# aschneuw/road-segmentation-unet

Measured on AMD Instinct MI355X. Metric: 388x388 patches/sec fwd+bwd (1/2/4/8 GPU) + conv MFMA % of peak, higher is better.
Workload: dtype bf16; 1 GPU; U-Net fwd+bwd+momentum step, num_layers=5 root_size=64 patch_size=388 input=572; batch_per_gpu=4, global_batch=4, parallelism=dp1

## Files before the change

road_segmentation_unet_amd/_lib.py:

```python
import ctypes
import os

_HERE = os.path.dirname(os.path.abspath(__file__))
LIB_PATH = os.environ.get("RSU_LIB_PATH") or os.path.join(_HERE, "librsu_hip.so")

_vp, _i, _l, _f, _sz, _u = ctypes.c_void_p, ctypes.c_int, ctypes.c_long, ctypes.c_float, ctypes.c_size_t, ctypes.c_uint


class RsuSrc(ctypes.Structure):
    _fields_ = [("ptr", _vp), ("H", _i), ("W", _i), ("C", _i), ("oy", _i), ("ox", _i)]


class RsuWgradJob(ctypes.Structure):
    _fields_ = [("kind", _i), ("src", RsuSrc), ("dz", _vp), ("dw", _vp), ("db", _vp), ("Ho", _i), ("Wo", _i),
                ("Cin_total", _i), ("ci_off", _i), ("Cout", _i), ("dil", _i)]


WGRAD_CONV3X3, WGRAD_CONVT2X2, WGRAD_GROUP_MAX = 0, 1, 16


class RsuPlanRow(ctypes.Structure):
    _fields_ = [(n, _i) for n in ("kind", "level", "Hin", "Win", "Cin", "Hout", "Wout", "Cout", "dilation", "nsrc")]


# ... 135 lines not shown
    "rsu_lovasz_ws_bytes": (_sz, [_i, _i, _i]),
    "rsu_lovasz_fwd": (_i, [_vp, _vp, _vp, _vp, _i, _i, _i, _vp]),
    "rsu_lovasz_fwd_bwd": (_i, [_vp, _vp, _f, _i, _vp, _vp, _vp, _i, _i, _i, _vp]),
}

SIGNATURES_COMPONENTS = {
    "rsu_components_ws_bytes": (_sz, [_i, _i, _i]),
    "rsu_components_label": (_i, [_vp, _f, _i, _i, _vp, _vp, _vp, _vp, _i, _i, _i, _vp]),
    "rsu_components_filter": (_i, [_vp, _f, _i, _i, _i, _vp, _vp, _vp, _i, _i, _i, _vp]),
    "rsu_components_pair_count": (_i, [_vp, _f, _vp, _i, _vp, _vp, _i, _i, _i, _vp]),
}

SIGNATURES_DISTANCE = {
    "rsu_distance_ws_bytes": (_sz, [_i, _i, _i]),
    "rsu_mask_distance": (_i, [_vp, _f, _vp, _vp, _vp, _vp, _i, _i, _i, _vp]),
    "rsu_distance_hist": (_i, [_vp, _f, _vp, _vp, _vp, _i, _i, _i, _vp]),
}

SIGNATURES_THIN = {
    "rsu_thin_ws_bytes": (_sz, [_i, _i, _i, _i]),
    "rsu_mask_thin": (_i, [_vp, _f, _vp, _i, _vp, _vp, _vp, _vp, _vp, _i, _i, _i, _vp]),
}

_lib = None


class RsuError(RuntimeError):
    pass


def lib():
    global _lib
    if _lib is None:
        if not os.path.exists(LIB_PATH):
            raise RsuError("HIP extension missing: %s (build it with `python -c 'import __graft_entry__ as g; g.build()'` "
                           "or `make -C road_segmentation_unet_amd/csrc`); there is no fallback path" % LIB_PATH)
        L = ctypes.CDLL(LIB_PATH)
        for name, (res, args) in list(SIGNATURES.items()) + list(SIGNATURES_OPTIM.items()) + list(SIGNATURES_LOSS.items()) \
                + list(SIGNATURES_CLDICE.items()) + list(SIGNATURES_LOVASZ.items()) + list(SIGNATURES_COMPONENTS.items()) \
                + list(SIGNATURES_DISTANCE.items()) + list(SIGNATURES_THIN.items()):
            fn = getattr(L, name)
            fn.restype = res
            fn.argtypes = args
        _lib = L
    return _lib


TUNE_OFF, TUNE_LOOKUP, TUNE_MEASURE = 0, 1, 2
EVAL_BINS = 256
BORDER_D2_INF, BORDER_MAX_SIDE = 0x7fffffff, 1024
CLIP_STATE_BYTES, CLIP_CLIPPED, CLIP_NONFINITE, GRAD_NORM_BLOCK_FLOATS = 32, 1, 2, 16384
GRAD_ACCUMULATE_BLOCK_FLOATS = 8192
DECAY_L2, DECAY_DECOUPLED = 0, 1
AFFINE_MAX_LAUNCH = 32
ELASTIC_MAX_LAUNCH, ELASTIC_MAX_GRID = 32, 16
JITTER_MAX_LAUNCH = 32
CLDICE_MAX_ITERS = 16
DIST_BINS, DIST_NONE, DIST_MAX_SIDE = 64, 0x7fffffff, 1024
THIN_MAX_SIDE, THIN_MAX_ITERS = 1024, 512
E2BIG = -7


def check(rc, what):
# ... 73 lines not shown
```

road_segmentation_unet_amd/csrc/igemm.h:

```cpp
#pragma once
#include "rsu_common.h"

struct IgSrc {
    const bf16_t* ptr;
    int H, W, C;
    int oy, ox;
};

struct IgFwdParams {
    IgSrc src[3];
    int nsrc;
    int nchunk[3];
    const bf16_t* wp;
    long wp_y_stride;
    int ntiles_w;
    int tile_off;
    const float* bias;
    bf16_t* out;
    const bf16_t* mask_src;
    bf16_t* pool_out;
    unsigned char* pool_code;
    const void* zero_page;
    int N, Hin, Win;
    int Ho, Wo;
// ... 30 lines not shown
hipError_t igemm_pp_finish_launch(int cfg, const IgFwdParams& p, hipStream_t st);

struct IgCtParams {
    const bf16_t* a;
    int Ca;
    int nchunk;
    int N, H, W;
    unsigned magic_hw, magic_w;
    const bf16_t* wp;
    long wp_phase_stride;
    int ntiles_w;
    const float* bias;
    bf16_t* out;
    int outC;
    int Cn;
    const bf16_t* mask_src;
    int ncob, nnb;
};
bool igemm_ct_supports(int mode, int N, int H, int W, int Ca, int Cn);
hipError_t igemm_ct_launch(int mode, const IgCtParams& p, int grid_x, hipStream_t st);
hipError_t conv_first_fwd_launch(const void* in16, const void* wp, int ntiles_w, const float* bias, void* y, int N, int H, int W, int Cout, int dil,
                                 int relu, int ncu, hipStream_t st, const float* x = nullptr, const float* cw = nullptr, const float* cb = nullptr);

struct IgWgradParams {
    const bf16_t* F;
    int Hf, Wf, Cf;
    IgSrc S;
    float* slab;
    float* bslab;
    float* sbslab;
    long slab_stride;
    int CsOut, CfOut, cs_off;
    const void* zero_page;
    int N, dil, stride;
    int nsplit, ntiles_total;
    int lsw;
    int nbuf, nsw;
    int dbg;
    TileGeo g;
};
enum { IGW_CFG_64x64 = 0, IGW_CFG_64x16 = 1, IGW_CFG_128x64 = 2, IGW_NCFG = 3 };
size_t igemm_wgrad_lds_bytes(int cfg, int npix_max, int nbuf);
int igemm_wgrad_nsw(int cfg, int npix_max);
int igemm_wgrad_tmk(int cfg);
int igemm_wgrad_cfb(int cfg);
int igemm_wgrad_csb(int cfg);
int igemm_wgrad_kgroups(int cfg);
hipError_t igemm_wgrad_launch(int cfg, int ntap, const IgWgradParams& p, int grid_x, int grid_y, int grid_z,
                              hipStream_t st);
bool igemm_wgt_supports(int N, int H, int W, int Cin, int Cout);
int igemm_wgt_blocks(int Cin, int Cout);
int igemm_wgt_tiles(int N, int H, int W);
hipError_t igemm_wgt_launch(const void* x, const void* dy, float* slab, float* sbslab, long slab_stride, int N, int H, int W, int Cin, int Cout,
                            int nsplit, hipStream_t st);
bool igemm_wg1_supports(int N, int H, int W, int Cout, int dil);
int igemm_wg1_blocks(int Cout);
int igemm_wg1_tiles(int N, int Ho, int Wo);
hipError_t igemm_wg1_launch(const void* in16, const void* dz, float* slab, float* bslab, long slab_stride, int N, int H, int W, int Cout, int dil,
                            int nsplit, hipStream_t st);
enum { IGW_FAM_WGPP3 = 0, IGW_FAM_WGPP4 = 1, IGW_FAM_WGPP5 = 2, IGW_FAM_WGPP6 = 3, IGW_FAM_WGP64_4 = 4, IGW_FAM_WGP64_5 = 5,
       IGW_FAM_GENERIC = 8  };
#define IGW_GROUP_MAX 16
// ... 22 lines not shown
```

road_segmentation_unet_amd/csrc/igemm_wgpp.hip:

```cpp
#include <type_traits>

#include "igemm_wgrad_body.h"

#define RSU_SENT 0x80000000u

namespace {
constexpr int sched_nph(int sch) { return sch >= 4 ? 1 : 2; }
constexpr int sched_count(int sch, int ph) {
    constexpr int T2[8] = {0, 3, 0, 3, 0, 3, 0, 0}, T1[4] = {3, 3, 3, 0};
    return sch >= 4 ? T1[ph] : T2[ph];
}
constexpr int sched_first(int sch, int ph) {
    int n = 0;
    for (int i = 0; i < ph; ++i) n += sched_count(sch, i);
    return n;
}
#ifndef WGPP_NT
#define WGPP_NT 0
#endif
#ifndef WG64_NT
#define WG64_NT 0
#endif
template <int NT = 0>
__device__ __forceinline__ void bdma16w(__amdgpu_buffer_rsrc_t rsrc, unsigned voff, unsigned soff, void* lds_wave_base) {
// ... 539 lines not shown
#pragma unroll
                for (int ct = 0; ct < CFT; ++ct) {
                    const int cf = cfb * 64 + ((ct + wcs) & 3) * 16 + 4 * g4;
                    if (cf >= p.Cf) continue;
                    float* dst = p.slab + (long)z * p.slab_stride + (((long)(T0 + t) * p.CsOut + p.cs_off + cs) * p.CfOut + cf);
                    *(f32x4*)dst = acc[t][ct];
                }
            }
        }
    };
    if (grp) {
        run(I1{});
    } else {
        run(I0{});
        bar();
    }
    asm volatile("s_waitcnt vmcnt(0)" ::: "memory");
}

#define WG_UNIT_FROM_GRID()                                                                                                                   \
    extern __shared__ __attribute__((aligned(16))) char smem[];                                                                              \
    __attribute__((address_space(3))) char* lds = (__attribute__((address_space(3))) char*)smem;                                             \
    const int lid = xcd_contiguous_id(blockIdx.x + gridDim.x * (blockIdx.y + gridDim.y * blockIdx.z), gridDim.x * gridDim.y * gridDim.z);  \
    const int cfb = lid % gridDim.x, csb = (lid / gridDim.x) % gridDim.y, z = lid / (gridDim.x * gridDim.y)
template <int LSW, int DBG, int SCH>
__global__ void __launch_bounds__(512) __attribute__((amdgpu_waves_per_eu(2, 2))) igemm_wgpp_kernel(const IgWgradParams p) {
    WG_UNIT_FROM_GRID();
    igemm_wgpp_body<LSW, DBG, SCH>(p, lds, cfb, csb, z, threadIdx.x);
}
template <int LSW>
__global__ void __launch_bounds__(512) __attribute__((amdgpu_waves_per_eu(2, 2))) igemm_wgp64_kernel(const IgWgradParams p) {
    WG_UNIT_FROM_GRID();
    igemm_wgp64_body<LSW>(p, lds, cfb, csb, z, threadIdx.x);
}

template <int FAM, class P>
__device__ __forceinline__ void wg_group_unit(const P& p, __attribute__((address_space(3))) char* lds, int cfb, int csb, int z, unsigned tid) {
    if constexpr (FAM == IGW_FAM_WGPP3) igemm_wgpp_body<3, 0, 4>(p, lds, cfb, csb, z, tid);
    else if constexpr (FAM == IGW_FAM_WGPP4) igemm_wgpp_body<4, 0, 4>(p, lds, cfb, csb, z, tid);
    else if constexpr (FAM == IGW_FAM_WGPP5) igemm_wgpp_body<5, 0, 4>(p, lds, cfb, csb, z, tid);
    else if constexpr (FAM == IGW_FAM_WGPP6) igemm_wgpp_body<6, 0, 4>(p, lds, cfb, csb, z, tid);
    else if constexpr (FAM == IGW_FAM_WGP64_4) igemm_wgp64_body<4>(p, lds, cfb, csb, z, tid);
    else if constexpr (FAM == IGW_FAM_WGP64_5) igemm_wgp64_body<5>(p, lds, cfb, csb, z, tid);
    else {
        constexpr int CFG = (FAM - IGW_FAM_GENERIC) >> 1, NTAP = ((FAM - IGW_FAM_GENERIC) & 1) ? 4 : 9, KW = NTAP == 4 ? 2 : 3;
        using C = WgCfg<CFG>;
        igemm_wgrad_body<C::WCF, C::WCS, C::CFT, C::CST, NTAP, KW, C::TMK, C::KG>(p, lds, cfb, csb, z, tid);
    }
}
__global__ void __launch_bounds__(512) __attribute__((amdgpu_waves_per_eu(2, 2))) igemm_wg_group_kernel(const IgWgGroupParams* table) {
    extern __shared__ __attribute__((aligned(16))) char smem[];
    __attribute__((address_space(3))) char* lds = (__attribute__((address_space(3))) char*)smem;
    {
        const unsigned state = IGW_GROUP_LDS_BYTES - 256 + (threadIdx.x >> 6) * 16;
        const u32x4 st0 = {(unsigned)__ldg(&table->wg_first[blockIdx.x]), (unsigned)__ldg(&table->wg_first[blockIdx.x + 1]),
                           (unsigned)(uintptr_t)table, (unsigned)((uintptr_t)table >> 32)};
// ... 125 lines not shown
```

road_segmentation_unet_amd/csrc/igemm_wgrad.hip:

```cpp
#include "igemm_wgrad_body.h"

template <int WCF, int WCS, int CFT, int CST, int NTAP, int KW, int TMK, int KG>
__global__ void __launch_bounds__(WCF* WCS * KG * 64) __attribute__((amdgpu_waves_per_eu(WCF* WCS* KG / 4, WCF* WCS* KG / 4)))
igemm_wgrad_kernel(const IgWgradParams p) {
    extern __shared__ __attribute__((aligned(16))) char smem[];
    __attribute__((address_space(3))) char* lds = (__attribute__((address_space(3))) char*)smem;
    const int lid = xcd_contiguous_id(blockIdx.x + gridDim.x * (blockIdx.y + gridDim.y * blockIdx.z), gridDim.x * gridDim.y * gridDim.z);
    const int cfb = lid % gridDim.x, csb = (lid / gridDim.x) % gridDim.y, z = lid / (gridDim.x * gridDim.y);
    igemm_wgrad_body<WCF, WCS, CFT, CST, NTAP, KW, TMK, KG>(p, lds, cfb, csb, z, threadIdx.x);
}

int igemm_wgrad_kgroups(int) { return 1; }
int igemm_wgrad_tmk(int) { return 128; }
int igemm_wgrad_cfb(int cfg) { return cfg == IGW_CFG_128x64 ? 128 : 64; }
int igemm_wgrad_csb(int cfg) { return cfg == IGW_CFG_64x16 ? 16 : 64; }

int igemm_wgrad_nsw(int cfg, int npix_max) {
    const int csb = igemm_wgrad_csb(cfg);
    const int ppp = 64 / (csb / 8);
    return ((npix_max + ppp - 1) / ppp + 7) / 8;
}
size_t igemm_wgrad_lds_bytes(int cfg, int npix_max, int nbuf) {
    const int csb = igemm_wgrad_csb(cfg);
    const size_t staging = (size_t)nbuf * igemm_wgrad_tmk(cfg) * 2 * igemm_wgrad_cfb(cfg) +
                           (size_t)nbuf * igemm_wgrad_nsw(cfg, npix_max) * 8 * 1024;
    const size_t reduce = cfg == IGW_CFG_128x64 ? 0 : (size_t)(9 * 64 * csb + 64 * csb) * 4;
    return staging > reduce ? staging : reduce;
}

template <int CFG, int NTAP, int KW>
static hipError_t wlaunch_one(const IgWgradParams& p, int gx, int gy, int gz, hipStream_t st) {
    using C = WgCfg<CFG>;
// ... 25 lines not shown
```

road_segmentation_unet_amd/csrc/igemm_wgrad_body.h:

```cpp
#pragma once
#include "igemm.h"


static __device__ __forceinline__ void bdma16(__amdgpu_buffer_rsrc_t rsrc, unsigned voff, unsigned soff, void* lds_wave_base) {
    __builtin_amdgcn_raw_ptr_buffer_load_lds(rsrc, (__attribute__((address_space(3))) void*)lds_wave_base, 16, voff, soff, 0, 0);
}
#define RSU_WG_WAIT(N) asm volatile("s_waitcnt vmcnt(%0)" ::"n"(N) : "memory")
#define RSU_SENT 0x80000000u

template <int WCF, int WCS, int CFT, int CST, int NTAP, int KW, int TMK, int KG, class P>
__device__ __forceinline__ void igemm_wgrad_body(const P& p, __attribute__((address_space(3))) char* lds, const int cfb, const int csb,
                                                 const int z, const unsigned tid) {
    constexpr int NW = WCF * WCS * KG;
    constexpr int KS = TMK / 32;
    constexpr int KSG = KS / KG;
    static_assert(KS % KG == 0, "k-steps must split evenly over the wave groups");
    constexpr int CFB = WCF * CFT * 16;
    constexpr int NPL = CFB / 64;
    constexpr int CSB = WCS * CST * 16;
    constexpr int KH = NTAP / KW;
    constexpr int SPITCH = CSB * 2;
    constexpr int LPP = CSB / 8;
    constexpr int PPP = 64 / LPP;
    constexpr int FPL = TMK * 128;
    constexpr int FBUF = NPL * FPL;
    static_assert(CFB % 64 == 0, "F block is a multiple of 64 channels");
    const int nbuf = p.nbuf, nsw = p.nsw;
    const int SBUF = nsw * NW * 1024;
    const int s_base = nbuf * FBUF;

    const int lane = tid & 63;
// ... 374 lines not shown
```

road_segmentation_unet_amd/csrc/rsu_api.hip:

```cpp
#include <array>
#include <atomic>
#include <cmath>
#include <cstdlib>
#include <cstring>
#include <algorithm>
#include <cstddef>
#include <map>
#include <mutex>
#include <vector>

#include "../../include/rsu.h"
#include "../../include/rsu_optim.h"
#include "../../include/rsu_loss.h"
#include "../../include/rsu_cldice.h"
#include "../../include/rsu_lovasz.h"
#include "../../include/rsu_components.h"
#include "../../include/rsu_distance.h"
#include "../../include/rsu_thin.h"
#include "affine_patches.h"
#include "color_jitter.h"
#include "border_map.h"
#include "elementwise.h"
#include "head.h"
#include "cldice.h"
#include "lovasz.h"
#include "components.h"
#include "distance.h"
#include "thin.h"
#include "optim.h"
#include "igemm.h"

static std::atomic<int> g_last_hip_error{0};
static void rsu_set_hip_error(int e) { g_last_hip_error.store(e); }

__device__ uint4 g_zero_page_dev[256];

static const void* zero_page() {
    static void* ptr[64] = {nullptr};
    int dev = 0;
    if (hipGetDevice(&dev) != hipSuccess || dev < 0 || dev >= 64) return nullptr;
    if (!ptr[dev]) {
// ... 949 lines not shown
    p.nsplit = pl.nsplit;
    p.ntiles_total = pl.ntiles;
    p.lsw = pl.lsw;
    p.nbuf = pl.nbuf;
    p.nsw = igemm_wgrad_nsw(cfg, pl.g.npix_max);
#ifdef RSU_DEV_KERNELS
    p.dbg = env_int("RSU_WG_DBG", 0);
#endif
    p.g = pl.g;
    w.cfg = cfg; w.ntap = ntap; w.gx = pl.gx; w.gy = pl.gy; w.ntiles = pl.ntiles;
    w.main_elems = (long)ntap * CsOut * CfOut;
    w.extra = db ? CfOut : (dbs ? rup(CsOut, 4) : 0);
    w.out = out; w.db = db; w.dbs = dbs; w.cs_cnt = S->C;
    return RSU_OK;
}
static void finish_wgrad(WgPrep& w, int nsplit, float* ws) {
    IgWgradParams& p = w.p;
    p.nsplit = nsplit;
    p.slab = nsplit == 1 ? w.out : ws;
    p.slab_stride = w.main_elems + w.extra;
    p.bslab = w.db ? (nsplit == 1 ? w.db : ws + w.main_elems) : nullptr;
    p.sbslab = w.dbs ? (nsplit == 1 ? w.dbs : ws + w.main_elems) : nullptr;
}
static int run_wgrad(int cfg, const void* F, int Hf, int Wf, int Cf, const rsu_src_t* S, float* out, float* ws, int CsOut, int CfOut,
                     int cs_off, int N, int ntap, int kw, int dil, int stride, int ncu_arg, hipStream_t st, float* db = nullptr, float* dbs = nullptr) {
    const int ncu = launch_ncu(ncu_arg);
    if (ncu < 0) return RSU_EINVAL;
    WgPrep w;
    const int rc = prep_wgrad(w, cfg, F, Hf, Wf, Cf, S, out, CsOut, CfOut, cs_off, N, ntap, kw, dil, stride, ncu, db, dbs);
    if (rc != RSU_OK) return rc;
    const int nslab = w.p.nsplit;
    finish_wgrad(w, nslab, ws);
    const IgWgradParams& p = w.p;
    if (env_int("RSU_WG_GEN", 2) >= 2 && igemm_wgpp_supports(w.cfg, ntap, p))
        HIP_CHECK_RET(igemm_wgpp_launch(p, w.gx, w.gy, nslab, st));
    else if (env_int("RSU_WG_GEN", 2) >= 2 && env_int("RSU_WG64", 1) && igemm_wgp64_supports(w.cfg, ntap, p))
        HIP_CHECK_RET(igemm_wgp64_launch(p, w.gx, w.gy, nslab, st));
    else
        HIP_CHECK_RET(igemm_wgrad_launch(w.cfg, ntap, p, w.gx, w.gy, nslab, st));
    if (nslab > 1) {
        HIP_CHECK_RET(ew_reduce_slabs(ws, out, db ? db : dbs, w.extra / 4, nslab, p.slab_stride, ntap, CsOut, cs_off, S->C, CfOut, st));
    }
    return RSU_OK;
}

extern "C" size_t rsu_conv2d_bwd_weight_ws_floats(int Cin_total, int src_C, int Cout) {
    return wgrad_max_slabs(IGW_CFG_64x64, Cout, src_C) * (9 * (size_t)Cin_total * Cout + Cout);
}
extern "C" int rsu_conv2d_bwd_weight(const rsu_src_t* src, const void* dz, float* dw, float* db, float* ws, int N, int Ho, int Wo,
                                     int Cin_total, int ci_off, int Cout, int dil, int ncu, rsu_stream_t stream) {
    if (!src || !src->ptr || !dz || !dw || !ws || src->C % 8 || Cout % 8 || ci_off + src->C > Cin_total || (dil != 1 && dil != 2))
        return RSU_EINVAL;
    if (src->oy < 0 || src->ox < 0 || src->oy + Ho + 2 * dil > src->H || src->ox + Wo + 2 * dil > src->W || Wo < 2) return RSU_EINVAL;
    return run_wgrad(IGW_CFG_64x64, dz, Ho, Wo, Cout, src, dw, ws, Cin_total, Cout, ci_off, N, 9, 3, dil, 1, ncu, (hipStream_t)stream, db);
}

extern "C" size_t rsu_convT2x2_bwd_weight_ws_floats(int Cin, int Cout) {
    size_t slabs = wgrad_max_slabs(IGW_CFG_64x64, Cin, Cout);
    const size_t wgt = (size_t)(256 / igemm_wgt_blocks(Cin, Cout));
    if (wgt > slabs) slabs = wgt;
    return slabs * (4 * (size_t)Cout * Cin + Cout);
}
extern "C" int rsu_convT2x2_bwd_weight(const void* x, const void* dy, float* dK, float* db, float* ws, int N, int H, int W, int Cin,
                                       int Cout, int ncu, rsu_stream_t stream) {
    if (!x || !dy || !dK || !ws || Cin % 8 || Cout % 8 || W < 2) return RSU_EINVAL;
    const int wgt_gen = env_int("RSU_WGT_GEN", 3);
    if (wgt_gen >= 2 && igemm_wgt_supports(N, H, W, Cin, Cout) && (wgt_gen >= 3 || launch_ncu(ncu) >= 192)) {
        const int n = launch_ncu(ncu);
        if (n < 0) return RSU_EINVAL;
        const int ntiles = igemm_wgt_tiles(N, H, W);
        int nsplit = n / igemm_wgt_blocks(Cin, Cout);
        nsplit = nsplit < 1 ? 1 : (nsplit > ntiles ? ntiles : nsplit);
        const long main_elems = 4l * Cout * Cin, extra = db ? rup(Cout, 4) : 0, stride = main_elems + extra;
        HIP_CHECK_RET(igemm_wgt_launch(x, dy, nsplit == 1 ? dK : ws, db ? (nsplit == 1 ? db : ws + main_elems) : nullptr, stride, N, H, W, Cin, Cout,
                                       nsplit, (hipStream_t)stream));
        if (nsplit > 1) HIP_CHECK_RET(ew_reduce_slabs(ws, dK, db, (int)(extra / 4), nsplit, stride, 4, Cout, 0, Cout, Cin, (hipStream_t)stream));
        return RSU_OK;
// ... 706 lines not shown
```

road_segmentation_unet_amd/unet.py:

```python
import ctypes
import math
import os

import numpy as np
import torch

from . import _lib
from ._lib import RsuSrc, RsuWgradJob, call
from .optim import (DECAY_MODES, DEFAULT_LR_SCHEDULE, EMA_SUFFIX, LR_SCHEDULES, OPTIMIZERS, OptimizerStep,
                    _PACK_CONV_BWD, _PACK_CONV_FIRST, _PACK_CONV_FWD, _PACK_CONVT_BWD, _PACK_CONVT_FWD, _accumulate_arg, _clip_arg,
                    _decay_args, _ema_arg, _int_arg, _ptr, adam_scalars, clip_scale, ema_decay_at, lr_at)
from .schedule import BackwardSchedule, cu_shares

NUM_CHANNELS = 3
NUM_LABELS = 2


def input_size_needed(output_size, num_layers):
    for i in range(num_layers - 1):
        assert output_size % 2 == 0, 'expand layer {} has size {} not divisible by 2' \
            .format(num_layers - i, output_size)
        output_size = (output_size + 4) / 2
    for i in range(num_layers - 1):
        output_size = (output_size + 4) * 2
# ... 22 lines not shown
    shapes += [("weight_output/kernel", (1, 1, nf, NUM_LABELS)), ("weight_output/bias", (NUM_LABELS,))]
    return shapes


def _is_dead(name, num_layers):
    return name.startswith("conv_dilut_%d/" % (num_layers - 1))


def glorot_uniform_params(num_layers, root_size, dilated_layers, seed):
    rng = np.random.RandomState(seed)
    out = {}
    for name, shp in param_shapes(num_layers, root_size, dilated_layers):
        if name.endswith("kernel"):
            recept = shp[0] * shp[1]
            limit = math.sqrt(6.0 / (recept * shp[2] + recept * shp[3]))
            out[name] = rng.uniform(-limit, limit, size=shp).astype(np.float32)
        else:
            out[name] = np.zeros(shp, np.float32)
    return out


def dropout_key_value(seed, site, global_step, micro_step=0):
    return (seed * 0x9E3779B9 + site * 0x85EBCA6B + global_step * 0xC2B2AE35 + micro_step * 0x27D4EB2F) & 0xFFFFFFFF


def _src(t, h, w):
    H, W, C = t.shape[1], t.shape[2], t.shape[3]
    return RsuSrc(t.data_ptr(), H, W, C, (H - h) // 2, (W - w) // 2)


class UNet(OptimizerStep):

    def __init__(self, num_layers, root_size, dilated_layers, batch_size, patch_size, device="cuda:0", params=None, seed=2017,
                 training=True, optimizer="momentum", class_weights=None, dice_weight=0.0, dice_smooth=1.0, border_weight=0.0, border_sigma=5.0,
                 clip_grad_norm=None, ema_decay=None, ema_warmup=True, accumulate_steps=None, weight_decay=None, weight_decay_mode="decoupled",
                 focal_gamma=0.0, cldice_weight=0.0, cldice_iters=10, cldice_smooth=1.0, lovasz_weight=0.0):
        self._init_optimizer(training, optimizer, clip_grad_norm, ema_decay, ema_warmup, accumulate_steps, weight_decay, weight_decay_mode)
        assert root_size % 8 == 0 and (root_size // 8) & (root_size // 8 - 1) == 0, "root_size must be 8 * 2^k for the HIP path"
        self.L, self.root, self.dilated = num_layers, root_size, bool(dilated_layers)
        self.B, self.P = batch_size, patch_size
        self.S = input_size_needed(patch_size, num_layers)
        self.device = torch.device(device)
        if self.device.type == "cuda":
            torch.cuda.set_device(self.device)
        self.training = training
        self.class_weights = class_weights
# ... 278 lines not shown
                h = (h - 4) // 2
                nf *= 2
        h = h - 4
        for i in range(L - 1):
            nf //= 2
            j = L + i
            self.act["up_%d" % i] = self._bf(B, 2 * h, 2 * h, nf)
            h = 2 * h
            self.act["c1_%d" % j] = self._bf(B, h - 2, h - 2, nf)
            self.act["c2_%d" % j] = self._bf(B, h - 4, h - 4, nf)
            h -= 4
        assert h == self.P, (h, self.P)
        self.last_name = "c2_%d" % (2 * L - 2) if L > 1 else "c2_0"
        self.prob = torch.zeros((B, self.P, self.P), dtype=torch.float32, device=dev)
        self.logits = torch.zeros((B, self.P, self.P, 2), dtype=torch.float32, device=dev)
        self.labels = torch.zeros((B, self.P, self.P), dtype=torch.int64, device=dev)
        self._loss_acc = torch.zeros(2, dtype=torch.float32, device=dev)
        self.loss_sum, self.weight_sum = self._loss_acc[0:1], self._loss_acc[1:2]
        self.dice_sums = torch.zeros(3, dtype=torch.float32, device=dev)
        self.eval_sums = torch.zeros(5, dtype=torch.float32, device=dev)
        self.eval_hist = torch.zeros((2, _lib.EVAL_BINS), dtype=torch.int64, device=dev)
        nk = int(_lib.lib().rsu_conv_splitk_ws_floats()) if os.environ.get("RSU_KSPLIT", "1") != "0" else 0
        self.sched.kws = torch.zeros(nk, dtype=torch.float32, device=dev) if nk else None
        self.sched.kws_side = [torch.zeros(nk, dtype=torch.float32, device=dev) for _ in self.wstreams] if (nk and self.dilated) else []
        if self.training:
            for k, t in self.act.items():
                if k.startswith("up_") or k.startswith("c") or k.startswith("d") or k.startswith("pool_"):
                    self.grad[k] = torch.zeros_like(t)
            for i in range(L - 1):
                up = self.act["up_%d" % i]
                self.grad["skip_%d" % i] = torch.zeros_like(up)
                if self.dilated:
                    self.grad["skipd_%d" % i] = torch.zeros_like(up)
            lib = _lib.lib()
            ws = [lib.rsu_head_ws_floats(B * self.P * self.P, self.root), lib.rsu_head_w_ws_floats(B * self.P * self.P, self.root),
                  lib.rsu_head_dice_ws_floats(B * self.P * self.P, self.root), lib.rsu_head_eval_ws_floats(B * self.P * self.P, self.root),
                  lib.rsu_conv_first_bwd_ws_floats(self.root)]
            for kind, n, s, segs in self._packed_kernels():
                if kind == _PACK_CONV_FWD:
                    for c in segs:
                        ws.append(lib.rsu_conv2d_bwd_weight_ws_floats(s[2], c, s[3]))
                    ws.append(lib.rsu_bias_grad_ws_floats(B * S * S, s[3]))
                elif kind == _PACK_CONVT_FWD:
                    ws.append(lib.rsu_convT2x2_bwd_weight_ws_floats(s[3], s[2]))
            ws.append(lib.rsu_wgrad_group_ws_floats())
            self.ws = torch.zeros(int(max(ws)) + 64, dtype=torch.float32, device=dev)
            self.sched.ws_side = [self.ws] + [torch.zeros_like(self.ws) for _ in self.wstreams[1:]]
            self.gfirst = torch.zeros((2, 9, 12, self.root), dtype=torch.float32, device=dev)
            if self._cldice_weight > 0.0:
                self._cldice_buffers()
            if self._lovasz_weight > 0.0:
                self._lovasz_buffers()
            if self.border_weight > 0.0:
                self.border_map = torch.zeros((B, self.P, self.P), dtype=torch.float32, device=dev)
                self._border_ws = torch.zeros(int(lib.rsu_border_map_ws_bytes(B, self.P, self.P)) // 4, dtype=torch.int32, device=dev)
            if os.environ.get("RSU_POOL_CODE", "1") == "1":
                for i in range(L - 1):
                    self.pool_code[i] = torch.zeros(self.act["pool_%d" % i].shape, dtype=torch.uint8, device=dev)

    def _conv_sources_c(self, name, shape):
        cin, cout = shape[2], shape[3]
        blk = int(name.split("/")[0].split("_")[-1]) if name.startswith("conv_") and not name.startswith("conv_dilut") else -1
        if name.endswith("conv1/kernel") and blk >= self.L:
            return [cout] * (3 if self.dilated else 2)
# ... 191 lines not shown
            self.eval_lovasz_sum.zero_()

    def evaluate_device(self):
        if not self.training:
            raise _lib.RsuError("evaluate_device needs a training net (labels and the head's workspace); a forward-only net has no loss")
        if self.keep != 1.0:
            raise _lib.RsuError("evaluate_device follows forward_device(keep=1.0): the activations in flight were made with dropout")
        if self._focal_gamma > 0.0:
            call("rsu_head_eval_focal", _ptr(self.act[self.last_name]), _ptr(self.w["weight_output/kernel"]), _ptr(self.w["weight_output/bias"]),
                 _ptr(self.labels), _ptr(self._class_w_dev), _ptr(self._head_pixel_weights()), self._focal_gamma, _ptr(self.prob),
                 _ptr(self.eval_sums), _ptr(self.eval_hist), _ptr(self.ws), self.B * self.P * self.P, self.root, self._stream())
        else:
            call("rsu_head_eval", _ptr(self.act[self.last_name]), _ptr(self.w["weight_output/kernel"]), _ptr(self.w["weight_output/bias"]),
                 _ptr(self.labels), _ptr(self._class_w_dev), _ptr(self._head_pixel_weights()), _ptr(self.prob), _ptr(self.eval_sums),
                 _ptr(self.eval_hist), _ptr(self.ws), self.B * self.P * self.P, self.root, self._stream())
        if self._cldice_weight > 0.0:
            self._cldice_buffers()
            self._cldice_fwd(self.eval_cldice_sums)
        if self._lovasz_weight > 0.0:
            self._lovasz_buffers()
            call("rsu_lovasz_fwd", _ptr(self.prob), _ptr(self.labels), _ptr(self.eval_lovasz_sum), _ptr(self._lovasz_ws), self.B, self.P,
                 self.P, self._stream())

    def _wgrad(self, name, srcs_t, dz, hout, dil=1, block_done=False):
        cout = dz.shape[3]
        cin_total = self.w[name + "/kernel"].shape[2]
        off = 0
        if self.sched.grouped:
            for t, win in srcs_t:
                db = self.g[name + "/bias"] if off == 0 else None
                job = RsuWgradJob(_lib.WGRAD_CONV3X3, _src(t, win, win), dz.data_ptr(), self.g[name + "/kernel"].data_ptr(),
                                  db.data_ptr() if db is not None else None, hout, hout, cin_total, off, cout, dil)
                self.sched.queue(job, 2.0 * self.B * hout * hout * cout * t.shape[3] * 9, (name, off))
                off += t.shape[3]
            if block_done:
                self.sched.block_done()
            return
        with self.sched.side() as ws:
            st = self._stream()
            for t, win in srcs_t:
                s = _src(t, win, win)
                db = _ptr(self.g[name + "/bias"]) if off == 0 else None
                fl = 2.0 * self.B * hout * hout * cout * t.shape[3] * 9
                self._timed("conv3x3_bwd_weight", fl, "rsu_conv2d_bwd_weight", ctypes.byref(s), _ptr(dz), _ptr(self.g[name + "/kernel"]), db,
                            _ptr(ws), self.B, hout, hout, cin_total, off, cout, dil, self.sched.ncu(), st)
                off += t.shape[3]

    def _wgradT(self, i, upin, dup, hh, nf):
        if self.sched.grouped:
            job = RsuWgradJob(_lib.WGRAD_CONVT2X2, RsuSrc(upin.data_ptr(), hh, hh, upin.shape[3], 0, 0), dup.data_ptr(),
                              self.g["up_conv_%d/kernel" % i].data_ptr(), self.g["up_conv_%d/bias" % i].data_ptr(), 0, 0, 0, 0, nf, 1)
            self.sched.queue(job, 0.0, ("up_conv_%d" % i, upin.data_ptr()), transposed=True)
            return
        with self.sched.side() as ws:
            call("rsu_convT2x2_bwd_weight", _ptr(upin), _ptr(dup), _ptr(self.g["up_conv_%d/kernel" % i]), _ptr(self.g["up_conv_%d/bias" % i]),
                 _ptr(ws), self.B, hh, hh, upin.shape[3], nf, self.sched.ncu(), self._stream())

    def _wgrad_first(self, name, dz, h, dil, where):
        with where as ws:
            call("rsu_conv_first_bwd_weight", _ptr(self.in16), _ptr(dz), _ptr(self.g[name + "/kernel"]), _ptr(self.gfirst[dil - 1]),
                 _ptr(self.g[name + "/bias"]), _ptr(ws), self.B, h, h, self.root, dil, self.sched.ncu(), self._stream())

    def _bwd_data(self, name, dz, dx, hin, relu_src=None, accumulate=0, src_index=0, dil=1):
        cout = self.w[name + "/kernel"].shape[3]
        cnt = dx.shape[3]
        ho = hin - 2 * dil
        kws = self.sched.kws_here()
        self._timed("conv3x3_bwd_data", 2.0 * self.B * ho * ho * cout * cnt * 9, "rsu_conv2d_bwd_data_k", _ptr(dz),
                    _ptr(self.pk[name + "/kernel", "bwd", src_index]), _ptr(dx), _ptr(relu_src), accumulate, self.B, hin, hin, cnt, 0, cnt,
# ... 71 lines not shown
            npix = B * self.P * self.P
            call("rsu_head_dice_sums", *head, _ptr(pixel_w), _ptr(self.prob), _ptr(self.dice_sums), _ptr(self.ws), npix, self.root, st)
            call("rsu_head_fwd_bwd_dice", *head, _ptr(self._class_w_dev), _ptr(pixel_w), _ptr(self.dice_sums), dice_scale,
                 self._dice_smooth, _ptr(self.prob), _ptr(self.loss_sum), _ptr(self.weight_sum), _ptr(g[self.last_name]),
                 _ptr(self.g["weight_output/kernel"]), _ptr(self.g["weight_output/bias"]), _ptr(self.ws), npix, self.root, inv_count, st)
        elif self.loss_is_weighted():
            call("rsu_head_fwd_bwd_w", _ptr(last), _ptr(self.w["weight_output/kernel"]), _ptr(self.w["weight_output/bias"]), _ptr(self.labels),
                 _ptr(self._class_w_dev), _ptr(pixel_w), _ptr(self.prob),
                 _ptr(self.loss_sum), _ptr(self.weight_sum), _ptr(g[self.last_name]), _ptr(self.g["weight_output/kernel"]),
                 _ptr(self.g["weight_output/bias"]), _ptr(self.ws), B * self.P * self.P, self.root, inv_count, st)
        else:
            call("rsu_head_fwd_bwd", _ptr(last), _ptr(self.w["weight_output/kernel"]), _ptr(self.w["weight_output/bias"]), _ptr(self.labels),
                 _ptr(self.prob), _ptr(self.loss_sum), _ptr(g[self.last_name]), _ptr(self.g["weight_output/kernel"]),
                 _ptr(self.g["weight_output/bias"]), _ptr(self.ws), B * self.P * self.P, self.root, inv_count, st)
        for i in reversed(range(L - 1)):
            j, lvl = L + i, L - 2 - i
            c1, c2, up = a["c1_%d" % j], a["c2_%d" % j], a["up_%d" % i]
            h = up.shape[1]
            nf = c2.shape[3]
            dz2, dz1 = g["c2_%d" % j], g["c1_%d" % j]
            self._wgrad("conv_%d/conv2" % j, [(c1, h - 2)], dz2, h - 4, block_done=True)
            self._bwd_data("conv_%d/conv2" % j, dz2, dz1, h - 2, relu_src=c1)
            srcs = [(a["c2_%d" % lvl], h)] + ([(a["d2_%d" % lvl], h)] if self.dilated else []) + [(up, h)]
            self._wgrad("conv_%d/conv1" % j, srcs, dz1, h - 2)
            self._bwd_data("conv_%d/conv1" % j, dz1, g["skip_%d" % i], h, src_index=0)
            if self.dilated:
                self._bwd_data("conv_%d/conv1" % j, dz1, g["skipd_%d" % i], h, src_index=1)
            dup = g["up_%d" % i]
            self._bwd_data("conv_%d/conv1" % j, dz1, dup, h, src_index=2 if self.dilated else 1)
            upin = a["c2_%d" % (j - 1)] if i > 0 else a["c2_%d" % (L - 1)]
            gin = g["c2_%d" % (j - 1)] if i > 0 else g["c2_%d" % (L - 1)]
            if keep < 1.0:
                upin = a["drop_%d" % i]
            hh = h // 2
            self._wgradT(i, upin, dup, hh, nf)
            call("rsu_convT2x2_bwd_data", _ptr(dup), _ptr(self.pk["up_conv_%d/kernel" % i, "bwd"]), _ptr(gin), _ptr(upin), float(np.float32(1.0) / np.float32(keep)), B, hh, hh,
                 upin.shape[3], nf, self.sched.ncu(), st)
            self._grads_ready("up_conv_%d/kernel" % i)
        for i in reversed(range(L)):
            c1, c2 = a["c1_%d" % i], a["c2_%d" % i]
            h = self.level_in[i]
            nf = c2.shape[3]
            dz2, dz1 = g["c2_%d" % i], g["c1_%d" % i]
            if i < L - 1:
                dec = L - 2 - i
                hs = a["up_%d" % dec].shape[1]
                call("rsu_pool_skip_relu_bwd_code", _ptr(c2), _ptr(self.pool_code.get(i)), _ptr(g["pool_%d" % i]), _ptr(g["skip_%d" % dec]), _ptr(dz2), B, h - 4, h - 4, nf, hs, hs,
                     keep, self.dropout_key(i + 1), st)
            self._wgrad("conv_%d/conv2" % i, [(c1, h - 2)], dz2, h - 4, block_done=i > 0 or self.dilated)
            self._bwd_data("conv_%d/conv2" % i, dz2, dz1, h - 2, relu_src=c1)
            if i > 0:
                pin = a["pool_%d" % (i - 1)]
                self._wgrad("conv_%d/conv1" % i, [(pin, h)], dz1, h - 2)
                self._bwd_data("conv_%d/conv1" % i, dz1, g["pool_%d" % (i - 1)], h)
            else:
                alone = not (self.dilated and L > 1)
                self.sched.flush(alone=alone)
                self._wgrad_first("conv_0/conv1", dz1, h, 1, self.sched.tail(alone))
            if self.dilated and i < L - 1:
                d1, d2 = a["d1_%d" % i], a["d2_%d" % i]
                dzd2, dzd1 = g["d2_%d" % i], g["d1_%d" % i]
                dec = L - 2 - i
                hs = a["up_%d" % dec].shape[1]
                call("rsu_pool_skip_relu_bwd", _ptr(d2), None, _ptr(g["skipd_%d" % dec]), _ptr(dzd2), B, h - 8, h - 8, nf, hs, hs, 1.0, 0, st)
                self._wgrad("conv_dilut_%d/atrous_conv2" % i, [(d1, h - 4)], dzd2, h - 8, dil=2, block_done=True)
                self._bwd_data("conv_dilut_%d/atrous_conv2" % i, dzd2, dzd1, h - 4, relu_src=d1, dil=2)
                if i > 0:
                    pin = a["pool_%d" % (i - 1)]
                    self._wgrad("conv_dilut_%d/atrous_conv1" % i, [(pin, h)], dzd1, h - 4, dil=2)
# ... 62 lines not shown
```

Measured before the change: 916.6 patches/s.

## Merge multi-source concat wgrad into one launch and optionally move skip bwd-data to side stream

Adds a concatenated-input weight-gradient entry point. A single implicit-GEMM wgrad launch now covers all concat sources (skip plus upsampled) of decoder conv1: each block picks its source from its csb index and writes into the right input-channel offset, replacing one launch and slab reduction per source. This is meant to cut launch count, reduce partial-slab traffic, and give a larger grid for better CU occupancy. A second, env-gated option (off by default) runs the skip-path bwd-data on the side stream with event synchronisation. The catch is extra per-block source-selection logic in the kernels and a larger workspace.

Measured after the change: 935.5 patches/s (median of 5 runs). Within noise of the previous version (+2.1%).

```diff
diff --git a/include/rsu_wgrad_cat.h b/include/rsu_wgrad_cat.h
--- /dev/null
+++ b/include/rsu_wgrad_cat.h
@@ -0,0 +1,20 @@
+#ifndef RSU_WGRAD_CAT_H_
+#define RSU_WGRAD_CAT_H_
+
+#include "rsu.h"
+
+#ifdef __cplusplus
+extern "C" {
+#endif
+
+#define RSU_WGRAD_CAT_MAX_SRC 3
+
+size_t rsu_conv2d_bwd_weight_cat_ws_floats(const int* src_C, int nsrc, int Cout);
+int rsu_conv2d_bwd_weight_cat(const rsu_src_t* srcs, int nsrc, const void* dz, float* dw, float* db, float* ws, int N, int Ho, int Wo,
+                              int Cin_total, int Cout, int dil, int ncu, rsu_stream_t stream);
+
+#ifdef __cplusplus
+}
+#endif
+
+#endif
diff --git a/road_segmentation_unet_amd/_lib.py b/road_segmentation_unet_amd/_lib.py
--- a/road_segmentation_unet_amd/_lib.py
+++ b/road_segmentation_unet_amd/_lib.py
@@ -181,6 +181,11 @@
     "rsu_mask_thin": (_i, [_vp, _f, _vp, _i, _vp, _vp, _vp, _vp, _vp, _i, _i, _i, _vp]),
 }
 
+SIGNATURES_WGRAD_CAT = {
+    "rsu_conv2d_bwd_weight_cat_ws_floats": (_sz, [_PI, _i, _i]),
+    "rsu_conv2d_bwd_weight_cat": (_i, [_PS, _i, _vp, _vp, _vp, _vp, _i, _i, _i, _i, _i, _i, _i, _vp]),
+}
+
 _lib = None
 
 
@@ -197,7 +202,7 @@
         L = ctypes.CDLL(LIB_PATH)
         for name, (res, args) in list(SIGNATURES.items()) + list(SIGNATURES_OPTIM.items()) + list(SIGNATURES_LOSS.items()) \
                 + list(SIGNATURES_CLDICE.items()) + list(SIGNATURES_LOVASZ.items()) + list(SIGNATURES_COMPONENTS.items()) \
-                + list(SIGNATURES_DISTANCE.items()) + list(SIGNATURES_THIN.items()):
+                + list(SIGNATURES_DISTANCE.items()) + list(SIGNATURES_THIN.items()) + list(SIGNATURES_WGRAD_CAT.items()):
             fn = getattr(L, name)
             fn.restype = res
             fn.argtypes = args
diff --git a/road_segmentation_unet_amd/csrc/igemm.h b/road_segmentation_unet_amd/csrc/igemm.h
--- a/road_segmentation_unet_amd/csrc/igemm.h
+++ b/road_segmentation_unet_amd/csrc/igemm.h
@@ -76,6 +76,11 @@
 hipError_t conv_first_fwd_launch(const void* in16, const void* wp, int ntiles_w, const float* bias, void* y, int N, int H, int W, int Cout, int dil,
                                  int relu, int ncu, hipStream_t st, const float* x = nullptr, const float* cw = nullptr, const float* cb = nullptr);
 
+struct IgWgSrc {
+    IgSrc S;
+    int cs_first, cs_off;
+};
+#define IGW_SRC_MAX 3
 struct IgWgradParams {
     const bf16_t* F;
     int Hf, Wf, Cf;
@@ -92,6 +97,8 @@
     int nbuf, nsw;
     int dbg;
     TileGeo g;
+    int nsrc;
+    IgWgSrc src[IGW_SRC_MAX];
 };
 enum { IGW_CFG_64x64 = 0, IGW_CFG_64x16 = 1, IGW_CFG_128x64 = 2, IGW_NCFG = 3 };
 size_t igemm_wgrad_lds_bytes(int cfg, int npix_max, int nbuf);
diff --git a/road_segmentation_unet_amd/csrc/igemm_wgpp.hip b/road_segmentation_unet_amd/csrc/igemm_wgpp.hip
--- a/road_segmentation_unet_amd/csrc/igemm_wgpp.hip
+++ b/road_segmentation_unet_amd/csrc/igemm_wgpp.hip
@@ -585,16 +585,18 @@
     extern __shared__ __attribute__((aligned(16))) char smem[];                                                                              \
     __attribute__((address_space(3))) char* lds = (__attribute__((address_space(3))) char*)smem;                                             \
     const int lid = xcd_contiguous_id(blockIdx.x + gridDim.x * (blockIdx.y + gridDim.y * blockIdx.z), gridDim.x * gridDim.y * gridDim.z);  \
-    const int cfb = lid % gridDim.x, csb = (lid / gridDim.x) % gridDim.y, z = lid / (gridDim.x * gridDim.y)
+    const int cfb = lid % gridDim.x, z = lid / (gridDim.x * gridDim.y);                                                                      \
+    int csb = (lid / gridDim.x) % gridDim.y;                                                                                                 \
+    const IgWgradParams q = igemm_wg_select_src(p, csb)
 template <int LSW, int DBG, int SCH>
 __global__ void __launch_bounds__(512) __attribute__((amdgpu_waves_per_eu(2, 2))) igemm_wgpp_kernel(const IgWgradParams p) {
     WG_UNIT_FROM_GRID();
-    igemm_wgpp_body<LSW, DBG, SCH>(p, lds, cfb, csb, z, threadIdx.x);
+    igemm_wgpp_body<LSW, DBG, SCH>(q, lds, cfb, csb, z, threadIdx.x);
 }
 template <int LSW>
 __global__ void __launch_bounds__(512) __attribute__((amdgpu_waves_per_eu(2, 2))) igemm_wgp64_kernel(const IgWgradParams p) {
     WG_UNIT_FROM_GRID();
-    igemm_wgp64_body<LSW>(p, lds, cfb, csb, z, threadIdx.x);
+    igemm_wgp64_body<LSW>(q, lds, cfb, csb, z, threadIdx.x);
 }
 
 template <int FAM, class P>
diff --git a/road_segmentation_unet_amd/csrc/igemm_wgrad.hip b/road_segmentation_unet_amd/csrc/igemm_wgrad.hip
--- a/road_segmentation_unet_amd/csrc/igemm_wgrad.hip
+++ b/road_segmentation_unet_amd/csrc/igemm_wgrad.hip
@@ -6,8 +6,10 @@
     extern __shared__ __attribute__((aligned(16))) char smem[];
     __attribute__((address_space(3))) char* lds = (__attribute__((address_space(3))) char*)smem;
     const int lid = xcd_contiguous_id(blockIdx.x + gridDim.x * (blockIdx.y + gridDim.y * blockIdx.z), gridDim.x * gridDim.y * gridDim.z);
-    const int cfb = lid % gridDim.x, csb = (lid / gridDim.x) % gridDim.y, z = lid / (gridDim.x * gridDim.y);
-    igemm_wgrad_body<WCF, WCS, CFT, CST, NTAP, KW, TMK, KG>(p, lds, cfb, csb, z, threadIdx.x);
+    const int cfb = lid % gridDim.x, z = lid / (gridDim.x * gridDim.y);
+    int csb = (lid / gridDim.x) % gridDim.y;
+    const IgWgradParams q = igemm_wg_select_src(p, csb);
+    igemm_wgrad_body<WCF, WCS, CFT, CST, NTAP, KW, TMK, KG>(q, lds, cfb, csb, z, threadIdx.x);
 }
 
 int igemm_wgrad_kgroups(int) { return 1; }
diff --git a/road_segmentation_unet_amd/csrc/igemm_wgrad_body.h b/road_segmentation_unet_amd/csrc/igemm_wgrad_body.h
--- a/road_segmentation_unet_amd/csrc/igemm_wgrad_body.h
+++ b/road_segmentation_unet_amd/csrc/igemm_wgrad_body.h
@@ -7,6 +7,27 @@
 }
 #define RSU_WG_WAIT(N) asm volatile("s_waitcnt vmcnt(%0)" ::"n"(N) : "memory")
 #define RSU_SENT 0x80000000u
+
+static __device__ __forceinline__ IgWgradParams igemm_wg_select_src(const IgWgradParams& p, int& csb) {
+    IgWgradParams q = p;
+    if (p.nsrc > 1) {
+        const int s = (p.nsrc > 2 && csb >= p.src[2].cs_first) ? 2 : (csb >= p.src[1].cs_first ? 1 : 0);
+        auto sgpr = [](int v) { return __builtin_amdgcn_readfirstlane(v); };
+#define RSU_WG_SEL(f) (s == 2 ? p.src[2].f : (s == 1 ? p.src[1].f : p.src[0].f))
+        const uintptr_t ptr = (uintptr_t)RSU_WG_SEL(S.ptr);
+        q.S.ptr = (const bf16_t*)(((uintptr_t)(unsigned)sgpr((int)(ptr >> 32)) << 32) | (uintptr_t)(unsigned)sgpr((int)ptr));
+        q.S.H = sgpr(RSU_WG_SEL(S.H));
+        q.S.W = sgpr(RSU_WG_SEL(S.W));
+        q.S.C = sgpr(RSU_WG_SEL(S.C));
+        q.S.oy = sgpr(RSU_WG_SEL(S.oy));
+        q.S.ox = sgpr(RSU_WG_SEL(S.ox));
+        q.cs_off = sgpr(RSU_WG_SEL(cs_off));
+        csb = sgpr(csb - RSU_WG_SEL(cs_first));
+#undef RSU_WG_SEL
+        if (s != 0) q.bslab = nullptr;
+    }
+    return q;
+}
 
 template <int WCF, int WCS, int CFT, int CST, int NTAP, int KW, int TMK, int KG, class P>
 __device__ __forceinline__ void igemm_wgrad_body(const P& p, __attribute__((address_space(3))) char* lds, const int cfb, const int csb,
diff --git a/road_segmentation_unet_amd/csrc/rsu_api.hip b/road_segmentation_unet_amd/csrc/rsu_api.hip
--- a/road_segmentation_unet_amd/csrc/rsu_api.hip
+++ b/road_segmentation_unet_amd/csrc/rsu_api.hip
@@ -17,6 +17,7 @@
 #include "../../include/rsu_components.h"
 #include "../../include/rsu_distance.h"
 #include "../../include/rsu_thin.h"
+#include "../../include/rsu_wgrad_cat.h"
 #include "affine_patches.h"
 #include "color_jitter.h"
 #include "border_map.h"
@@ -1012,6 +1013,12 @@
     p.bslab = w.db ? (nsplit == 1 ? w.db : ws + w.main_elems) : nullptr;
     p.sbslab = w.dbs ? (nsplit == 1 ? w.dbs : ws + w.main_elems) : nullptr;
 }
+static hipError_t launch_wgrad(const WgPrep& w, int gy, int nslab, hipStream_t st) {
+    if (env_int("RSU_WG_GEN", 2) >= 2 && igemm_wgpp_supports(w.cfg, w.ntap, w.p)) return igemm_wgpp_launch(w.p, w.gx, gy, nslab, st);
+    if (env_int("RSU_WG_GEN", 2) >= 2 && env_int("RSU_WG64", 1) && igemm_wgp64_supports(w.cfg, w.ntap, w.p))
+        return igemm_wgp64_launch(w.p, w.gx, gy, nslab, st);
+    return igemm_wgrad_launch(w.cfg, w.ntap, w.p, w.gx, gy, nslab, st);
+}
 static int run_wgrad(int cfg, const void* F, int Hf, int Wf, int Cf, const rsu_src_t* S, float* out, float* ws, int CsOut, int CfOut,
                      int cs_off, int N, int ntap, int kw, int dil, int stride, int ncu_arg, hipStream_t st, float* db = nullptr, float* dbs = nullptr) {
     const int ncu = launch_ncu(ncu_arg);
@@ -1022,15 +1029,54 @@
     const int nslab = w.p.nsplit;
     finish_wgrad(w, nslab, ws);
     const IgWgradParams& p = w.p;
-    if (env_int("RSU_WG_GEN", 2) >= 2 && igemm_wgpp_supports(w.cfg, ntap, p))
-        HIP_CHECK_RET(igemm_wgpp_launch(p, w.gx, w.gy, nslab, st));
-    else if (env_int("RSU_WG_GEN", 2) >= 2 && env_int("RSU_WG64", 1) && igemm_wgp64_supports(w.cfg, ntap, p))
-        HIP_CHECK_RET(igemm_wgp64_launch(p, w.gx, w.gy, nslab, st));
-    else
-        HIP_CHECK_RET(igemm_wgrad_launch(w.cfg, ntap, p, w.gx, w.gy, nslab, st));
+    HIP_CHECK_RET(launch_wgrad(w, w.gy, nslab, st));
     if (nslab > 1) {
         HIP_CHECK_RET(ew_reduce_slabs(ws, out, db ? db : dbs, w.extra / 4, nslab, p.slab_stride, ntap, CsOut, cs_off, S->C, CfOut, st));
     }
+    return RSU_OK;
+}
+static int run_wgrad_cat(const rsu_src_t* srcs, int nsrc, const void* dz, float* dw, float* db, float* ws, int N, int Ho, int Wo,
+                         int Cin_total, int Cout, int dil, int ncu_arg, hipStream_t st) {
+    const int ncu = launch_ncu(ncu_arg);
+    if (ncu < 0) return RSU_EINVAL;
+    WgPrep w;
+    bool merged = nsrc > 1;
+    if (merged) {
+        for (int s = 1; s < nsrc; ++s)
+            if ((long)N * srcs[s].H * srcs[s].W * srcs[s].C * 2 >= 0x7ffffff0L) return RSU_E2BIG;
+        const int rc = prep_wgrad(w, IGW_CFG_64x64, dz, Ho, Wo, Cout, &srcs[0], dw, Cin_total, Cout, 0, N, 9, 3, dil, 1, ncu, db, nullptr);
+        if (rc != RSU_OK) return rc;
+        const int csb = igemm_wgrad_csb(w.cfg);
+        for (int s = 0; s < nsrc; ++s) merged = merged && srcs[s].C % csb == 0;
+    }
+    if (!merged) {
+        int off = 0;
+        for (int s = 0; s < nsrc; ++s) {
+            const int rc = run_wgrad(IGW_CFG_64x64, dz, Ho, Wo, Cout, &srcs[s], dw, ws, Cin_total, Cout, off, N, 9, 3, dil, 1, ncu_arg, st,
+                                     s == 0 ? db : nullptr);
+            if (rc != RSU_OK) return rc;
+            off += srcs[s].C;
+        }
+        return RSU_OK;
+    }
+    IgWgradParams& p = w.p;
+    const int csb = igemm_wgrad_csb(w.cfg);
+    int gy = 0, off = 0;
+    p.nsrc = nsrc;
+    for (int s = 0; s < nsrc; ++s) {
+        IgWgSrc& e = p.src[s];
+        e.S.ptr = (const bf16_t*)srcs[s].ptr;
+        e.S.H = srcs[s].H; e.S.W = srcs[s].W; e.S.C = srcs[s].C; e.S.oy = srcs[s].oy; e.S.ox = srcs[s].ox;
+        e.cs_first = gy;
+        e.cs_off = off;
+        gy += srcs[s].C / csb;
+        off += srcs[s].C;
+    }
+    int nslab = ncu / (w.gx * gy);
+    nslab = nslab < 1 ? 1 : (nslab > w.ntiles ? w.ntiles : nslab);
+    finish_wgrad(w, nslab, ws);
+    HIP_CHECK_RET(launch_wgrad(w, gy, nslab, st));
+    if (nslab > 1) HIP_CHECK_RET(ew_reduce_slabs(ws, dw, db, w.extra / 4, nslab, p.slab_stride, 9, Cin_total, 0, Cin_total, Cout, st));
     return RSU_OK;
 }
 
@@ -1043,6 +1089,40 @@
         return RSU_EINVAL;
     if (src->oy < 0 || src->ox < 0 || src->oy + Ho + 2 * dil > src->H || src->ox + Wo + 2 * dil > src->W || Wo < 2) return RSU_EINVAL;
     return run_wgrad(IGW_CFG_64x64, dz, Ho, Wo, Cout, src, dw, ws, Cin_total, Cout, ci_off, N, 9, 3, dil, 1, ncu, (hipStream_t)stream, db);
+}
+
+static_assert(RSU_WGRAD_CAT_MAX_SRC == IGW_SRC_MAX, "rsu_wgrad_cat.h and igemm.h must agree on the number of sources");
+extern "C" size_t rsu_conv2d_bwd_weight_cat_ws_floats(const int* src_C, int nsrc, int Cout) {
+    if (!src_C || nsrc < 1 || nsrc > IGW_SRC_MAX) return 0;
+    int Cin_total = 0;
+    for (int s = 0; s < nsrc; ++s) Cin_total += src_C[s];
+    size_t need = 0;
+    for (int s = 0; s < nsrc; ++s) {
+        const size_t n = rsu_conv2d_bwd_weight_ws_floats(Cin_total, src_C[s], Cout);
+        need = n > need ? n : need;
+    }
+    const int shapes[2] = {IGW_CFG_64x64, wgrad_pick_cfg(IGW_CFG_64x64, Cout)};
+    for (int k = 0; k < 2; ++k) {
+        int gy = 0;
+        for (int s = 0; s < nsrc; ++s) gy += cdiv(src_C[s], igemm_wgrad_csb(shapes[k]));
+        const int split = 256 / (cdiv(Cout, igemm_wgrad_cfb(shapes[k])) * (gy < 1 ? 1 : gy));
+        const size_t n = (size_t)(split < 1 ? 1 : split) * (9 * (size_t)Cin_total * Cout + Cout);
+        need = n > need ? n : need;
+    }
+    return need;
+}
+extern "C" int rsu_conv2d_bwd_weight_cat(const rsu_src_t* srcs, int nsrc, const void* dz, float* dw, float* db, float* ws, int N, int Ho,
+                                         int Wo, int Cin_total, int Cout, int dil, int ncu, rsu_stream_t stream) {
+    if (!srcs || nsrc < 1 || nsrc > IGW_SRC_MAX || !dz || !dw || !ws || Cout % 8 || (dil != 1 && dil != 2) || Wo < 2) return RSU_EINVAL;
+    long sum = 0;
+    for (int s = 0; s < nsrc; ++s) {
+        const rsu_src_t& c = srcs[s];
+        if (!c.ptr || c.C < 8 || c.C % 8) return RSU_EINVAL;
+        if (c.oy < 0 || c.ox < 0 || c.oy + Ho + 2 * dil > c.H || c.ox + Wo + 2 * dil > c.W) return RSU_EINVAL;
+        sum += c.C;
+    }
+    if (sum != Cin_total) return RSU_EINVAL;
+    return run_wgrad_cat(srcs, nsrc, dz, dw, db, ws, N, Ho, Wo, Cin_total, Cout, dil, ncu, (hipStream_t)stream);
 }
 
 extern "C" size_t rsu_convT2x2_bwd_weight_ws_floats(int Cin, int Cout) {
diff --git a/road_segmentation_unet_amd/unet.py b/road_segmentation_unet_amd/unet.py
--- a/road_segmentation_unet_amd/unet.py
+++ b/road_segmentation_unet_amd/unet.py
@@ -68,6 +68,15 @@
 
 def dropout_key_value(seed, site, global_step, micro_step=0):
     return (seed * 0x9E3779B9 + site * 0x85EBCA6B + global_step * 0xC2B2AE35 + micro_step * 0x27D4EB2F) & 0xFFFFFFFF
+
+
+_WG_CAT_DEFAULT = "1"
+_SKIP_SIDE_DEFAULT = ""
+
+
+def _skip_side_stages(L):
+    spec = os.environ.get("RSU_SKIP_SIDE", _SKIP_SIDE_DEFAULT)
+    return frozenset(int(v) for v in spec.split(",") if v.strip() and 0 <= int(v) < L - 1)
 
 
 def _src(t, h, w):
@@ -392,7 +401,10 @@
         self.eval_hist = torch.zeros((2, _lib.EVAL_BINS), dtype=torch.int64, device=dev)
         nk = int(_lib.lib().rsu_conv_splitk_ws_floats()) if os.environ.get("RSU_KSPLIT", "1") != "0" else 0
         self.sched.kws = torch.zeros(nk, dtype=torch.float32, device=dev) if nk else None
-        self.sched.kws_side = [torch.zeros(nk, dtype=torch.float32, device=dev) for _ in self.wstreams] if (nk and self.dilated) else []
+        self._skip_side = _skip_side_stages(L) if (self.training and self.wstreams) else frozenset()
+        self._skip_events, self._skip_pending = {}, set()
+        self.sched.kws_side = ([torch.zeros(nk, dtype=torch.float32, device=dev) for _ in self.wstreams]
+                               if (nk and (self.dilated or self._skip_side)) else [])
         if self.training:
             for k, t in self.act.items():
                 if k.startswith("up_") or k.startswith("c") or k.startswith("d") or k.startswith("pool_"):
@@ -410,6 +422,8 @@
                 if kind == _PACK_CONV_FWD:
                     for c in segs:
                         ws.append(lib.rsu_conv2d_bwd_weight_ws_floats(s[2], c, s[3]))
+                    if len(segs) > 1:
+                        ws.append(lib.rsu_conv2d_bwd_weight_cat_ws_floats((ctypes.c_int * len(segs))(*segs), len(segs), s[3]))
                     ws.append(lib.rsu_bias_grad_ws_floats(B * S * S, s[3]))
                 elif kind == _PACK_CONVT_FWD:
                     ws.append(lib.rsu_convT2x2_bwd_weight_ws_floats(s[3], s[2]))
@@ -647,7 +661,7 @@
             call("rsu_lovasz_fwd", _ptr(self.prob), _ptr(self.labels), _ptr(self.eval_lovasz_sum), _ptr(self._lovasz_ws), self.B, self.P,
                  self.P, self._stream())
 
-    def _wgrad(self, name, srcs_t, dz, hout, dil=1, block_done=False):
+    def _wgrad(self, name, srcs_t, dz, hout, dil=1, block_done=False, also=None):
         cout = dz.shape[3]
         cin_total = self.w[name + "/kernel"].shape[2]
         off = 0
@@ -663,13 +677,21 @@
             return
         with self.sched.side() as ws:
             st = self._stream()
-            for t, win in srcs_t:
-                s = _src(t, win, win)
-                db = _ptr(self.g[name + "/bias"]) if off == 0 else None
-                fl = 2.0 * self.B * hout * hout * cout * t.shape[3] * 9
-                self._timed("conv3x3_bwd_weight", fl, "rsu_conv2d_bwd_weight", ctypes.byref(s), _ptr(dz), _ptr(self.g[name + "/kernel"]), db,
-                            _ptr(ws), self.B, hout, hout, cin_total, off, cout, dil, self.sched.ncu(), st)
-                off += t.shape[3]
+            if len(srcs_t) > 1 and os.environ.get("RSU_WG_CAT", _WG_CAT_DEFAULT) != "0":
+                arr = (RsuSrc * len(srcs_t))(*[_src(t, win, win) for t, win in srcs_t])
+                fl = 2.0 * self.B * hout * hout * cout * cin_total * 9
+                self._timed("conv3x3_bwd_weight", fl, "rsu_conv2d_bwd_weight_cat", arr, len(srcs_t), _ptr(dz), _ptr(self.g[name + "/kernel"]),
+                            _ptr(self.g[name + "/bias"]), _ptr(ws), self.B, hout, hout, cin_total, cout, dil, self.sched.ncu(), st)
+            else:
+                for t, win in srcs_t:
+                    s = _src(t, win, win)
+                    db = _ptr(self.g[name + "/bias"]) if off == 0 else None
+                    fl = 2.0 * self.B * hout * hout * cout * t.shape[3] * 9
+                    self._timed("conv3x3_bwd_weight", fl, "rsu_conv2d_bwd_weight", ctypes.byref(s), _ptr(dz), _ptr(self.g[name + "/kernel"]), db,
+                                _ptr(ws), self.B, hout, hout, cin_total, off, cout, dil, self.sched.ncu(), st)
+                    off += t.shape[3]
+            if also is not None:
+                also()
 
     def _wgradT(self, i, upin, dup, hh, nf):
         if self.sched.grouped:
@@ -787,8 +809,18 @@
             self._wgrad("conv_%d/conv2" % j, [(c1, h - 2)], dz2, h - 4, block_done=True)
             self._bwd_data("conv_%d/conv2" % j, dz2, dz1, h - 2, relu_src=c1)
             srcs = [(a["c2_%d" % lvl], h)] + ([(a["d2_%d" % lvl], h)] if self.dilated else []) + [(up, h)]
-            self._wgrad("conv_%d/conv1" % j, srcs, dz1, h - 2)
-            self._bwd_data("conv_%d/conv1" % j, dz1, g["skip_%d" % i], h, src_index=0)
+            if i in self._skip_side and self.sched.streams and not self.sched.grouped:
+                def skip_on_side(i=i, j=j, dz1=dz1, h=h):
+                    self._bwd_data("conv_%d/conv1" % j, dz1, g["skip_%d" % i], h, src_index=0)
+                    ev = self._skip_events.get(i)
+                    if ev is None:
+                        ev = self._skip_events[i] = torch.cuda.Event()
+                    ev.record(torch.cuda.current_stream(self.device))
+                    self._skip_pending.add(i)
+                self._wgrad("conv_%d/conv1" % j, srcs, dz1, h - 2, also=skip_on_side)
+            else:
+                self._wgrad("conv_%d/conv1" % j, srcs, dz1, h - 2)
+                self._bwd_data("conv_%d/conv1" % j, dz1, g["skip_%d" % i], h, src_index=0)
             if self.dilated:
                 self._bwd_data("conv_%d/conv1" % j, dz1, g["skipd_%d" % i], h, src_index=1)
             dup = g["up_%d" % i]
@@ -810,6 +842,9 @@
             if i < L - 1:
                 dec = L - 2 - i
                 hs = a["up_%d" % dec].shape[1]
+                if dec in self._skip_pending:
+                    self._skip_pending.discard(dec)
+                    torch.cuda.current_stream(self.device).wait_event(self._skip_events[dec])
                 call("rsu_pool_skip_relu_bwd_code", _ptr(c2), _ptr(self.pool_code.get(i)), _ptr(g["pool_%d" % i]), _ptr(g["skip_%d" % dec]), _ptr(dz2), B, h - 4, h - 4, nf, hs, hs,
                      keep, self.dropout_key(i + 1), st)
             self._wgrad("conv_%d/conv2" % i, [(c1, h - 2)], dz2, h - 4, block_done=i > 0 or self.dilated)
```
